# team-charls/charls

Measured on AMD Instinct MI355X. Metric: MPixels/s encode+decode, 4096x4096 8-bit gray, bit-exact vs CharLS, higher is better.
Workload: dtype u8

## Files before the change

charls_amd/csrc/device/pipeline_common.hip:

```cpp
#pragma once
#include <hip/hip_runtime.h>

#include "knobs.h"
#include "scan_model.h"


namespace jls {
namespace pipe {

constexpr int kChains = 367;
constexpr int kRegularChains = 365;
constexpr int kInterruptChain = 365;
constexpr int kZeroContextChain = 366;
constexpr uint32_t kGradientTable = 512;
constexpr uint32_t kNoSlot = 0xFFFFFFFFu;
constexpr uint16_t kNoEvent = 0xFFFF;
constexpr uint32_t kPackBlock = 4096;
constexpr uint32_t kStatusInvalid = 1u;
constexpr uint32_t kChainPad = 16;
constexpr uint32_t kChainSlack = kChains * kChainPad + 64;

struct Work
{
    uint32_t* raw;
    uint64_t raw_words;
    uint64_t* total_bits;
    uint32_t* status;
    uint32_t* stuff_tables;
};

JLS_DEV uint32_t coded_lines(const ScanDesc& d)
{
    return d.interleave_mode == 1 ? d.height * (uint32_t)d.components : d.height;
}
JLS_DEV bool sign_fits_record(const ScanDesc& d)
{
    return d.bits_per_sample <= 15;
}
JLS_DEV uint32_t line_step(const ScanDesc& d)
{
    return d.interleave_mode == 1 ? (uint32_t)d.components : 1u;
}

template <typename S>
JLS_DEV void load_pixel(const ScanDesc& d, uint32_t y, uint32_t x, int mask, int out[4]);

template <typename S, int ILV>
JLS_DEV int load_sample(const ScanDesc& d, uint32_t line, uint32_t x, int mask)
{
    if (ILV == 1)
    {
        int px[4];
        load_pixel<S>(d, line / (uint32_t)d.components, x, mask, px);
        return px[line % (uint32_t)d.components];
    }
    const S* row = reinterpret_cast<const S*>(d.pixels + (size_t)line * d.pixel_stride);
    return (int)row[x] & mask;
}

JLS_DEV uint32_t line_samples(const ScanDesc& d)
{
    return d.interleave_mode == 2 ? d.width * (uint32_t)d.components : d.width;
}

template <typename S>
JLS_DEV void load_pixel(const ScanDesc& d, uint32_t y, uint32_t x, int mask, int out[4])
{
    const S* px = reinterpret_cast<const S*>(d.pixels + (size_t)y * d.pixel_stride) + (size_t)x * d.components;
    for (int c = 0; c < d.components; ++c)
        out[c] = (int)px[c] & mask;
    if (d.color_transformation != 0)
    {
        unsigned t[3];
        hp_forward(d.color_transformation, sizeof(S) == 2, out[0], out[1], out[2], t);
        out[0] = (int)t[0];
        out[1] = (int)t[1];
        out[2] = (int)t[2];
    }
}

typedef uint32_t u32x4 __attribute__((vector_size(16)));

struct CodeWord
{
    uint64_t bits;
    int len;
};

JLS_DEV CodeWord golomb_word(const Traits& t, int k, int m, int limit)
// ... 119 lines not shown
```

charls_amd/csrc/device/scan_model.h:

```cpp
#pragma once
#include <hip/hip_runtime.h>

#include "scan_types.h"

namespace jls {

#define JLS_DEV __device__ __forceinline__

#define JLS_LOCKSTEP() __builtin_amdgcn_wave_barrier()
#ifdef JLS_EMULATED
#define JLS_LOCKSTEP_STORES() __builtin_amdgcn_wave_barrier()
#else
#define JLS_LOCKSTEP_STORES() ((void)0)
#endif

#ifdef JLS_PATH_PROFILE
extern "C" unsigned long long jls_path_counts[32];
#define JLS_PATH(n) do { if (threadIdx.x == 0) ++jls_path_counts[n]; } while (0)
#define JLS_PATH_ADD(n, v) do { if (threadIdx.x == 0) jls_path_counts[n] += (unsigned long long)(v); } while (0)
#else
#define JLS_PATH(n) ((void)0)
#define JLS_PATH_ADD(n, v) ((void)0)
#endif

#ifndef JLS_GLOBAL_AS
#define JLS_GLOBAL_AS __attribute__((address_space(1)))
#endif

#ifndef JLS_DYNAMIC_LDS
#define JLS_DYNAMIC_LDS(name) extern __shared__ __attribute__((aligned(16))) unsigned char name[]
#endif

JLS_DEV uint32_t uniform(uint32_t v)
{
    return (uint32_t)__builtin_amdgcn_readfirstlane((int)v);
}

JLS_DEV uint32_t from_lane(uint32_t v, int l)
{
    return (uint32_t)__builtin_amdgcn_readlane((int)v, l);
}

#ifndef JLS_EMULATED
JLS_DEV int med3(int a, int b, int c)
{
    int r;
    asm("v_med3_i32 %0, %1, %2, %3" : "=v"(r) : "v"(a), "v"(b), "v"(c));
    return r;
}
JLS_DEV int med3s(int a, int b, int c_scalar)
{
    int r;
    asm("v_med3_i32 %0, %1, %2, %3" : "=v"(r) : "v"(a), "v"(b), "s"(c_scalar));
    return r;
}
#else
JLS_DEV int med3(int a, int b, int c)
{
    const int lo = a < b ? a : b, hi = a < b ? b : a;
    return c < lo ? lo : (c > hi ? hi : c);
// ... 112 lines not shown
                 : "s"(busy), "s"(ok)
                 : "scc");
    return ticker;
}
JLS_DEV uint32_t opaque(uint32_t v)
{
    asm volatile("" : "+v"(v));
    return v;
}
JLS_DEV uint32_t float_bits(uint32_t v)
{
    return __float_as_uint((float)v);
}
#define JLS_LDS_AS __attribute__((address_space(3)))
JLS_DEV uint32_t lds_address(const void* p)
{
    return (uint32_t)(uintptr_t)(const JLS_LDS_AS void*)p;
}
template <typename T>
JLS_DEV T lds_load(uint32_t address)
{
    return *(const JLS_LDS_AS T*)(uintptr_t)address;
}
template <typename T>
JLS_DEV void lds_store(uint32_t address, T v)
{
    *(JLS_LDS_AS T*)(uintptr_t)address = v;
}
JLS_DEV uint64_t load_relaxed(const uint64_t* p)
{
    return __hip_atomic_load(p, __ATOMIC_RELAXED, __HIP_MEMORY_SCOPE_AGENT);
}
JLS_DEV void store_relaxed(uint64_t* p, uint64_t v)
{
    __hip_atomic_store(p, v, __ATOMIC_RELAXED, __HIP_MEMORY_SCOPE_AGENT);
}
JLS_DEV uint32_t funnel_shift(uint32_t hi, uint32_t lo, uint32_t shift)
{
    return __builtin_amdgcn_alignbit(hi, lo, shift);
}
#else
JLS_DEV LaneMask lanes_where(bool p)
{
    return __ballot(p);
}
JLS_DEV bool lane_of(LaneMask m)
{
    return ((m >> emu::lane_id()) & 1ull) != 0;
}
JLS_DEV uint32_t value_of_lowest_lane(LaneMask m, uint32_t v)
{
    return (uint32_t)__builtin_amdgcn_readlane((int)v, __builtin_ctzll(m));
}
JLS_DEV int mad24(int a, int b, int c)
{
    return a * b + c;
}
JLS_DEV uint32_t pack_bytes(uint32_t s0, uint32_t s1)
{
    return (s1 & 0xFFu) | ((s0 & 0xFFu) << 8);
}
JLS_DEV uint32_t bit_field(uint32_t v, uint32_t offset, uint32_t width)
{
    return (v >> offset) & ((1u << width) - 1u);
}
JLS_DEV int sign_extend(int v, int bits)
// ... 324 lines not shown
```

charls_amd/csrc/device/tile_pipeline.hip:

```cpp
#pragma once
#include <hip/hip_runtime.h>

#include <algorithm>
#include <cstdlib>

#include "pipeline_common.hip"

namespace jls {
namespace tile {

using pipe::kChains;
using pipe::kInterruptChain;
using pipe::kNoEvent;
using pipe::kStatusInvalid;
using pipe::kZeroContextChain;


constexpr uint32_t kMaxTileSamples = 8192;
constexpr uint32_t kTileLines = 16;
constexpr uint32_t kSegments = 16;
constexpr uint32_t kThreads = 512;
constexpr uint32_t kWaves = kThreads / 64;
constexpr uint32_t kPackThreads = 512;
constexpr uint16_t kNoLocalSlot = 0xFFFF;
// ... 229 lines not shown
            all_a += na;
            all_b += nb;
        }
        a[half] = before_a + incl_a - a[half];
        b[half] = before_b + incl_b - b[half];
        carry_a += all_a;
        carry_b += all_b;
    }
}

template <typename S, int ILV>
struct Samples
{
    const ScanDesc& d;
    const S* rows;
    uint32_t first_line;
    int mask;
    JLS_DEV int operator()(uint32_t line, uint32_t x) const
    {
        static_assert(ILV == 0, "planar scans only");
        return (int)rows[(size_t)(line + 1 - first_line) * d.width + x] & mask;
    }
};

template <typename S, int ILV>
JLS_DEV void stage_lines(const ScanDesc& d, const TileGeometry& g, S* rows)
{
    const uint32_t width = g.width;
    const uint32_t bytes = width * (uint32_t)sizeof(S);
    const uint32_t first = g.first_line == 0 ? 1u : 0u;
    if (first)
        for (uint32_t x = threadIdx.x; x < width; x += blockDim.x)
            rows[x] = 0;
    const uint8_t* from = d.pixels + (size_t)(g.first_line + first - 1) * d.pixel_stride;
    uint8_t* to = reinterpret_cast<uint8_t*>(rows) + (size_t)first * bytes;
    const uint32_t lines = g.tile_lines + 1 - first;
    if (((reinterpret_cast<uintptr_t>(from) | d.pixel_stride | bytes) & 3u) == 0 && (reinterpret_cast<uintptr_t>(to) & 3u) == 0)
    {
        const uint32_t words_per_line = bytes / 4, total = lines * words_per_line;
        constexpr int kMost = (kMaxTileSamples * 2 / 4 + kThreads - 1) / kThreads;
        const uint32_t step_lines = kThreads / words_per_line, step_words = kThreads % words_per_line;
        uint32_t line = threadIdx.x / words_per_line, word = threadIdx.x % words_per_line;
        uint32_t held[kMost];
#pragma unroll
        for (int j = 0; j < kMost; ++j)
        {
            held[j] = line < lines ? reinterpret_cast<const uint32_t*>(from + (size_t)line * d.pixel_stride)[word] : 0u;
            line += step_lines;
            word += step_words;
            if (word >= words_per_line)
            {
                word -= words_per_line;
                ++line;
            }
        }
#pragma unroll
        for (int j = 0; j < kMost; ++j)
        {
            const uint32_t i = threadIdx.x + (uint32_t)j * kThreads;
            if (i < total)
                reinterpret_cast<uint32_t*>(to)[i] = held[j];
        }
        for (uint32_t i = threadIdx.x + kMost * kThreads; i < total; i += kThreads)
        {
            const uint32_t l2 = i / words_per_line, w2 = i - l2 * words_per_line;
            reinterpret_cast<uint32_t*>(to)[i] = reinterpret_cast<const uint32_t*>(from + (size_t)l2 * d.pixel_stride)[w2];
        }
    }
    else
        for (uint32_t r = 0; r < lines; ++r)
        {
            const S* from1 = reinterpret_cast<const S*>(from + (size_t)r * d.pixel_stride);
            S* to1 = reinterpret_cast<S*>(to + (size_t)r * bytes);
            for (uint32_t x = threadIdx.x; x < width; x += blockDim.x)
                to1[x] = from1[x];
        }
}

JLS_HOST_DEV_EARLY uint32_t sort_segments(uint32_t lines_per_tile)
{
    return lines_per_tile >= kWaves ? lines_per_tile : lines_per_tile * (kWaves / lines_per_tile);
}

struct TileLds
{
    uint32_t rows, keys, masks, table, end;
};
template <typename S, int ILV>
JLS_DEV TileLds tile_lds(uint32_t width, uint32_t lines_per_tile, bool with_keys)
{
    auto up = [](uint32_t v) { return (v + 15u) & ~15u; };
    TileLds l;
    const uint32_t chunks = (width + 63) / 64;
    l.rows = 0;
    l.keys = up((lines_per_tile + 1) * width * (uint32_t)sizeof(S));
    l.masks = l.keys + (with_keys ? up(lines_per_tile * width * 2u) : 0u);
    l.table = l.masks + up(lines_per_tile * chunks * 16u);
    l.end = l.table;
    return l;
}

template <typename S, int ILV>
__global__ void __launch_bounds__(kThreads) analyze_tiles(const ScanDesc* __restrict__ descs, const Work* __restrict__ works)
{
    JLS_DYNAMIC_LDS(smem);
// ... 45 lines not shown
                if (y >= step)
                {
                    rb = sample(y - step, x);
                    rc = x > 0 ? sample(y - step, x - 1) : edge_c;
                    rd = sample(y - step, x + 1 < width ? x + 1 : width - 1);
                }
                else
                    rc = x > 0 ? 0 : edge_c;
                const int qs = sizeof(S) == 1
                                   ? ((int)s_grad[rd - rb + 255] * 9 + (int)s_grad[rb - rc + 255]) * 9 + (int)s_grad[rc - ra + 255] - 364
                                   : context_id(t, ra, rb, rc, rd);
                const int sg = qs >> 31;
                const int ctx = (qs ^ sg) - sg;
                s_key[r * width + x] = (uint16_t)(ctx | ((sg & 1) << 9));
                eq = v == ra;
                q0 = qs == 0;
            }
            const unsigned long long m_eq = __ballot(eq);
            const unsigned long long m_q0 = __ballot(q0);
            if (lane == 0)
            {
                s_eq[r * chunks + k] = m_eq;
                s_q0[r * chunks + k] = m_q0;
            }
        }
    }
    __syncthreads();
    for (uint32_t sgm = wave; sgm < g.segments; sgm += kWaves)
    {
        const uint32_t r = sgm / g.pieces, piece = sgm % g.pieces;
        const uint32_t y = g.first_line + r;
        const uint32_t k0 = piece * g.chunks_per_piece;
        const uint32_t k1 = k0 + g.chunks_per_piece < chunks ? k0 + g.chunks_per_piece : chunks;
        uint16_t* key_row = w.keyinv + (size_t)y * width;
        unsigned long long carry = 0;
        for (uint32_t k = 0; k < k1; ++k)
        {
            const unsigned long long a = s_eq[r * chunks + k];
            const unsigned long long b = a & s_q0[r * chunks + k];
            const unsigned long long sum = a + b + carry;
            const unsigned long long st = sum ^ a ^ b;
            carry = (((a & b) | ((a | b) & st)) >> 63) & 1ull;
            const uint32_t x = k * 64 + lane;
            if (k >= k0 && x < width)
            {
                const bool s = (st >> lane) & 1ull;
                const bool q0 = (s_q0[r * chunks + k] >> lane) & 1ull;
                const bool eq = (a >> lane) & 1ull;
                uint16_t key = s_key[r * width + x];
                if (!(s || q0))
                    atomicAdd(&s_hist[key & 0x1FF], 1u);
                else if (s && eq)
                    key = kNoEvent;
                else if (s)
                {
                    key = (uint16_t)kInterruptChain;
                    atomicAdd(&s_hist[kInterruptChain], 1u);
                }
                else
                {
                    key = 0;
                    atomicAdd(&s_hist[0], 1u);
                }
                key_row[x] = key;
            }
        }
    }
    __syncthreads();
    for (uint32_t c = threadIdx.x; c < (uint32_t)kChains; c += kThreads)
        w.seg[(size_t)tile * kChains + c] = s_hist[c];
}

constexpr uint32_t kPlanThreads = 384;
JLS_DEV void plan_group(const ScanDesc& d, const Work& w, uint32_t g, uint32_t& t0, uint32_t& t1)
{
    const uint32_t tiles = scan_tiles(d, w);
    const uint32_t per_group = (tiles + kPlanGroups - 1) / kPlanGroups;
    t0 = g * per_group < tiles ? g * per_group : tiles;
    t1 = t0 + per_group < tiles ? t0 + per_group : tiles;
}
__global__ void __launch_bounds__(kPlanThreads) sum_chains(const ScanDesc* __restrict__ descs, const Work* __restrict__ works)
{
    const ScanDesc d = descs[blockIdx.y];
    const Work w = works[blockIdx.y];
    const uint32_t g = blockIdx.x, c = threadIdx.x;
    if (c >= (uint32_t)kChains)
        return;
    uint32_t t0, t1;
    plan_group(d, w, g, t0, t1);
    uint32_t sum = 0;
    for (uint32_t t = t0; t < t1; ++t)
        sum += w.seg[(size_t)t * kChains + c];
    w.plan_part[g * kChains + c] = sum * (c == 0 ? w.run_slots : 1u);
}
__global__ void __launch_bounds__(kPlanThreads) plan_chains(const ScanDesc* __restrict__ descs, const Work* __restrict__ works)
{
    __shared__ uint32_t s_base[kChains + 1];
    const Work w = works[blockIdx.x];
    uint32_t total = 0;
    if (threadIdx.x < (uint32_t)kChains)
    {
        const uint32_t c = threadIdx.x;
        for (uint32_t g = 0; g < kPlanGroups; ++g)
// ... 96 lines not shown
    static JLS_DEV int which(uint32_t v) { return (int)((v >> (kRunBits + kErrBits)) & 1u); }
    static JLS_DEV uint32_t component(uint32_t v) { return (v >> (is_end_of_line(v) ? 15u : kRunBits + kErrBits + 1)) & 3u; }
};

template <typename S, int ILV>
__global__ void __launch_bounds__(kThreads) sort_tiles(const ScanDesc* __restrict__ descs, const Work* __restrict__ works)
{
    JLS_DYNAMIC_LDS(smem);
    const ScanDesc d = descs[blockIdx.y];
    const Work w = works[blockIdx.y];
    const Traits t = make_traits(d);
    const uint32_t tile = tile_of_block(blockIdx.x, scan_tiles(d, w));
    if (tile >= scan_tiles(d, w))
        return;
    const TileGeometry g = tile_geometry(d, w, tile);
    constexpr uint32_t step = 1;
    const int lane = threadIdx.x & 63, wave = threadIdx.x >> 6;
    const uint32_t width = g.width, chunks = g.chunks;
    const TileLds lds = tile_lds<S, ILV>(width, w.lines_per_tile, false);
    S* s_rows = reinterpret_cast<S*>(smem + lds.rows);
    uint64_t* s_noev = reinterpret_cast<uint64_t*>(smem + lds.masks);
    uint32_t* s_lead = reinterpret_cast<uint32_t*>(s_noev + (size_t)w.lines_per_tile * chunks);
    uint32_t* s_segoff = reinterpret_cast<uint32_t*>(smem + lds.table);
    uint32_t* s_tileoff = s_segoff + sort_segments(w.lines_per_tile) * kChains;
    uint32_t* s_count = s_tileoff + kChains + 1;
    uint32_t* s_global = s_count + kChains + 1;
    uint32_t* s_tmp = s_global + kChains + 1;
    uint32_t* s_same = s_tmp + 16;
    uint32_t* s_rowbase = s_same + kWaves * (kChains + 1);
    uint16_t* s_rowchain = reinterpret_cast<uint16_t*>(s_rowbase + kChains + 1);
    Slot<S>* s_stage = reinterpret_cast<Slot<S>*>(s_rowbase + kChains + 1 + kRowChainWords);
    const int mask = (1 << d.bits_per_sample) - 1;
    const Samples<S, ILV> sample{d, s_rows, g.first_line, mask};
    const uint16_t* key_tile = w.keyinv + (size_t)g.first_line * width;

    JLS_PHASE_BEGIN();
    stage_lines<S, ILV>(d, g, s_rows);
    JLS_PHASE(0);
    for (uint32_t i = threadIdx.x; i < g.segments * (uint32_t)kChains; i += kThreads)
        s_segoff[i] = 0;
    for (uint32_t i = threadIdx.x; i < kWaves * ((uint32_t)kChains + 1); i += kThreads)
        s_same[i] = 0;
    __syncthreads();
    JLS_PHASE(1);
    for (uint32_t sgm = wave; sgm < g.segments; sgm += kWaves)
    {
        const uint32_t r = sgm / g.pieces, piece = sgm % g.pieces;
        const uint32_t k0 = piece * g.chunks_per_piece;
        const uint32_t k1 = k0 + g.chunks_per_piece < chunks ? k0 + g.chunks_per_piece : chunks;
        for (uint32_t kb = k0; kb < k1; kb += 16)
        {
            uint16_t held[16];
#pragma unroll
            for (int j = 0; j < 16; ++j)
            {
                const uint32_t x = (kb + j) * 64 + lane;
                held[j] = kb + j < k1 && x < width ? key_tile[(size_t)r * width + x] : kNoEvent;
            }
#pragma unroll
            for (int j = 0; j < 16; ++j)
            {
                const uint32_t k = kb + j;
                if (k < k1)
                {
                    const uint32_t x = k * 64 + lane;
                    const uint16_t key = held[j];
                    if (x < width && key != kNoEvent)
                        atomicAdd(&s_segoff[sgm * kChains + (key & 0x1FF)], (key & 0x1FF) == 0 ? run_slots_of<S>() : 1u);
                    const unsigned long long m = __ballot(x < width && key == kNoEvent);
                    if (lane == 0)
                        s_noev[r * chunks + k] = m;
                }
            }
        }
    }
    JLS_PHASE(2);
    __syncthreads();
    JLS_PHASE(3);
    for (uint32_t r = (uint32_t)wave; r < g.tile_lines; r += kWaves)
    {
        uint32_t behind = 0;
        for (uint32_t k0 = (chunks - 1) / 64 * 64;; k0 -= 64)
        {
            const uint32_t k = k0 + (uint32_t)lane;
            const unsigned long long m = k < chunks ? s_noev[r * chunks + k] : 0ull;
            const bool full = m == ~0ull;
            const uint32_t own = full ? 64u : (uint32_t)__ffsll(~m) - 1;
            const unsigned long long rest = __ballot(full) >> lane;
            const uint32_t ones = rest == ~0ull ? 64u : (uint32_t)__ffsll(~rest) - 1;
            const uint32_t next = __shfl(own, (int)((lane + ones) & 63u));
            const uint32_t lead = 64u * ones + ((uint32_t)lane + ones < 64u ? next : behind);
            if (k < chunks)
                s_lead[r * (chunks + 1) + k] = lead;
            behind = __shfl(lead, 0);
            if (k0 == 0)
                break;
        }
        if (lane == 0)
            s_lead[r * (chunks + 1) + chunks] = 0;
    }
    {
        static_assert(kChains <= kThreads, "a chain per thread");
        const uint32_t c = threadIdx.x;
        const bool chain = c < (uint32_t)kChains;
        uint32_t n = 0;
        if (chain)
            for (uint32_t sgm = 0; sgm < g.segments; ++sgm)
                n += s_segoff[sgm * kChains + c];
        const uint32_t rows = chain && c != (uint32_t)kInterruptChain ? (n + 63) / 64 : 0u;
        uint32_t off[2] = {n, 0}, row_base[2] = {rows, 0};
        block_exclusive_scan_pair(off, row_base, kChains, s_tmp);
        if (chain)
        {
            s_tileoff[c] = off[0];
            s_count[c] = n;
            s_global[c] = w.seg[(size_t)tile * kChains + c];
            uint32_t running = off[0];
            for (uint32_t sgm = 0; sgm < g.segments; ++sgm)
            {
                const uint32_t m = s_segoff[sgm * kChains + c];
                s_segoff[sgm * kChains + c] = running;
                running += m;
            }
            s_rowbase[c] = row_base[0];
            for (uint32_t j = 0; j < rows; ++j)
                s_rowchain[row_base[0] + j] = (uint16_t)c;
            if (c == (uint32_t)kChains - 1)
                s_rowbase[kChains] = row_base[0] + rows;
        }
    }
    JLS_PHASE(4);
    __syncthreads();
    JLS_PHASE(5);
    for (uint32_t sgm = wave; sgm < g.segments; sgm += kWaves)
    {
        const uint32_t r = sgm / g.pieces, piece = sgm % g.pieces;
        const uint32_t y = g.first_line + r;
        const uint32_t k0 = piece * g.chunks_per_piece;
        const uint32_t k1 = k0 + g.chunks_per_piece < chunks ? k0 + g.chunks_per_piece : chunks;
        uint32_t* segoff = s_segoff + sgm * kChains;
        uint32_t* same_of = s_same + (uint32_t)wave * (kChains + 1);
        uint16_t* inv_row = w.keyinv + (size_t)y * width;
        auto key_at = [&](uint32_t k) -> uint16_t {
            const uint32_t x = k * 64 + lane;
            return k < k1 && x < width ? inv_row[x] : kNoEvent;
        };
        uint16_t key_1 = key_at(k0), key_2 = key_at(k0 + 1);
        const S* cur = s_rows + (r + 1) * width;
        const int edge_a = y >= step ? sample(y - step, 0) : 0;
        const int edge_c = y >= 2 * step ? (r >= 1 ? sample(y - 2 * step, 0) : pipe::load_sample<S, 0>(d, y - 2, 0, mask)) : 0;
        const uint32_t lane_bit = 1u << (lane & 31), below = lane_bit - 1u;
        const bool upper = lane >= 32;
        for (uint32_t k = k0; k < k1; ++k)
        {
            const uint32_t x = k * 64 + lane;
            const bool inside = x < width;
            const uint16_t key = key_1;
            key_1 = key_2;
            key_2 = key_at(k + 2);
            const bool has = key != kNoEvent;
            const uint32_t chain = key & 0x1FFu;
            if (has && !upper)
                atomicOr(&same_of[chain], lane_bit);
            JLS_LOCKSTEP();
            const uint32_t lo = has ? same_of[chain] : 0u;
            JLS_LOCKSTEP();
            if (has && !upper)
                same_of[chain] = 0;
            JLS_LOCKSTEP();
            if (has && upper)
                atomicOr(&same_of[chain], lane_bit);
            JLS_LOCKSTEP();
            const uint32_t hi = has ? same_of[chain] : 0u;
            const uint32_t base = has ? segoff[chain] : 0u;
            JLS_LOCKSTEP();
            if (has && upper)
                same_of[chain] = 0;
            const uint32_t rank = upper ? (uint32_t)__popc(lo) + (uint32_t)__popc(hi & below) : (uint32_t)__popc(lo & below);
            const uint32_t per_event = chain == 0 ? run_slots_of<S>() : 1u;
            if (has && rank == 0)
                segoff[chain] = base + ((uint32_t)__popc(lo) + (uint32_t)__popc(hi)) * per_event;
            JLS_LOCKSTEP();
            const uint32_t slot = base + rank * per_event;
            uint32_t record = 0;
            if (inside)
            {
                const int v = (int)cur[x] & mask;
                const int ra = x > 0 ? (int)cur[x - 1] & mask : edge_a;
                const int rb = (int)(cur - width)[x] & mask;
                const int rc = x > 0 ? (int)(cur - width)[x - 1] & mask : edge_c;
                record = make_record<S>(v, med3(ra + rb - rc, ra, rb), (key >> 9) & 1, t.maxval);
            }
            if (__any(has && chain == 0))
            {
                if (has && chain == 0)
                {
                    const int v = sample(y, x);
                    const int ra = x > 0 ? sample(y, x - 1) : edge_a;
                    uint32_t run = 0;
                    if (v == ra)
                    {
                        const unsigned long long after = lane == 63 ? 0ull : s_noev[r * chunks + k] >> (lane + 1);
                        const uint32_t rest = 63u - (uint32_t)lane;
                        uint32_t n = (uint32_t)__ffsll(~after) - 1;
                        if (n >= rest)
                            n = rest + s_lead[r * (chunks + 1) + k + 1];
                        run = 1 + n;
                    }
                    const uint32_t xi = x + run;
                    if (xi >= width)
                        record = RunRecord<S>::end_of_line(run, 0u);
                    else
                    {
                        const int xv = sample(y, xi);
                        const int ia = xi > 0 ? sample(y, xi - 1) : edge_a;
                        const int ib = y >= step ? sample(y - step, xi) : 0;
                        const int which = ia == ib ? 1 : 0;
                        const int err = which ? error_value(t, xv - ia) : error_value(t, (xv - ib) * ((ib - ia) < 0 ? -1 : 1));
                        record = RunRecord<S>::interrupted(run, err, which, 0u);
                    }
                }
            }
            if (has)
            {
                if (run_slots_of<S>() == 2 && chain == 0)
                {
                    s_stage[slot] = (Slot<S>)(record & 0xFFFFu);
                    s_stage[slot + 1] = (Slot<S>)(record >> 16);
                }
                else
                    s_stage[slot] = (Slot<S>)record;
            }
            if (inside)
                inv_row[x] = has ? (uint16_t)slot : kNoLocalSlot;
        }
    }
    JLS_PHASE(6);
    __syncthreads();
    JLS_PHASE(7);
    const uint32_t total_rows = s_rowbase[kChains];
    constexpr int kRows = 4;
    for (uint32_t q0 = (uint32_t)wave * kRows; q0 < total_rows; q0 += kWaves * kRows)
    {
        uint32_t to[kRows];
        Slot<S> held[kRows];
        bool live[kRows];
#pragma unroll
        for (int j = 0; j < kRows; ++j)
        {
            const uint32_t q = q0 + (uint32_t)j;
            const uint32_t c = q < total_rows ? s_rowchain[q] : 0u;
            const uint32_t i = (q - s_rowbase[c]) * 64 + (uint32_t)lane;
            live[j] = q < total_rows && i < s_count[c];
            to[j] = s_global[c] + i;
            held[j] = live[j] ? s_stage[s_tileoff[c] + i] : (Slot<S>)0;
        }
#pragma unroll
        for (int j = 0; j < kRows; ++j)
            if (live[j])
                rec_slots<S>(w)[to[j]] = held[j];
    }
    JLS_PHASE(8);
}

}
}
#include "tile_pixel_mode.hip"
namespace jls {
namespace tile {

struct Chain
{
    int a, b, c, n;
    uint32_t bad;
};

JLS_DEV int chain_n_before(uint32_t i, uint32_t reset)
{
    if (reset == 0 || i < reset)
        return (int)(i + 1);
    const uint32_t half = reset >> 1, period = reset - half;
    return (int)(half + 1 + (i - reset) % period);
}

template <typename S>
JLS_DEV Slot<S> code_event(Chain& s, uint32_t rec, const Traits& t)
{
    int err;
    if (sizeof(S) == 1)
    {
        const int px = med3(s.c + (int)(rec >> 8), 0, t.maxval);
        err = sign_extend((int)(rec & 0xFFu) - px, t.bpp);
    }
// ... 792 lines not shown
    const uint32_t codes = (uint32_t)stage_bytes(tile_capacity, sample_bytes);
    const uint32_t head = ((codes + 3u) & ~3u) + 4 * ((uint32_t)kChains + 1) * 4 + kPackThreads * 4 + 16 * 4 + kRowChainWords * 4;
    return (head + 15u) & ~15u;
}

JLS_HOST_DEV uint32_t pack_bits_words(uint32_t tile_capacity, int32_t bits_per_sample)
{
    const uint32_t limit = 2u * (uint32_t)(bits_per_sample + (bits_per_sample > 8 ? bits_per_sample : 8));
    return tile_capacity * limit / 32 + 2;
}

JLS_DEV void expand_code(uint32_t word, uint64_t& bits, int& len)
{
    if (word & kRunTag)
    {
        const int ones = (int)((word >> 25) & 63u), tail_len = (int)((word >> 20) & 31u);
        bits = ((((uint64_t)1 << ones) - 1ull) << tail_len) | (uint64_t)(word & 0xFFFFFu);
        len = ones + tail_len;
    }
    else
    {
        bits = word & 0xFFFFFFu;
        len = (int)(word >> 24);
    }
}

JLS_DEV uint32_t shifted_word(const uint32_t* bits, uint32_t i, uint32_t head, uint32_t carry)
{
    if (head == 0)
        return bits[i];
    return (i == 0 ? carry : bits[i - 1] << (32u - head)) | (bits[i] >> head);
}

struct __attribute__((packed)) UnalignedQuadPair
{
    uint64_t lo, hi;
};
template <typename S>
__global__ void __launch_bounds__(kPackThreads) pack_tiles(const ScanDesc* __restrict__ descs, const Work* __restrict__ works)
{
    JLS_DYNAMIC_LDS(smem);
    constexpr bool kNarrow = sizeof(Slot<S>) == 2;
    const ScanDesc d = descs[blockIdx.y];
    const Work w = works[blockIdx.y];
    const uint32_t tile = blockIdx.x;
    const uint32_t tiles = scan_tiles(d, w);
    if (tile >= tiles)
        return;
    const uint32_t tile_capacity = w.tile_capacity;
    const uint32_t threads = blockDim.x;
    const uint32_t per_thread = ((tile_capacity + threads - 1) / threads + 7u) & ~7u;
    const int lane = threadIdx.x & 63, wave = threadIdx.x >> 6;
    const uint32_t kPackWaves = threads / 64;
    Slot<S>* s_code = reinterpret_cast<Slot<S>*>(smem);
    const uint32_t code_bytes = (uint32_t)stage_bytes(tile_capacity, (uint32_t)sizeof(S));
    uint32_t* s_tileoff = reinterpret_cast<uint32_t*>(smem + ((code_bytes + 3u) & ~3u));
    uint32_t* s_count = s_tileoff + kChains + 1;
    uint32_t* s_global = s_count + kChains + 1;
    uint32_t* s_scan = s_global + kChains + 1;
    uint32_t* s_tmp = s_scan + kPackThreads;
    uint32_t* s_rowbase = s_tmp + 16;
    uint16_t* s_rowchain = reinterpret_cast<uint16_t*>(s_rowbase + kChains + 1);
    uint32_t* s_bits = reinterpret_cast<uint32_t*>(smem + pack_bits_offset(tile_capacity, (uint32_t)sizeof(S)));
    const TileSpan span = tile_span(d, w, tile);
    const uint32_t tile_samples = span.count;
    const uint16_t* inv = w.keyinv + span.first;

    constexpr int kGroups = (int)(kMaxTileSamples / kPackThreads / 8);
    uint4 mine[kGroups];
    JLS_PHASE_BEGIN();
#pragma unroll
    for (int q = 0; q < kGroups; ++q)
    {
        const uint32_t at = threadIdx.x * per_thread + (uint32_t)q * 8;
        mine[q] = make_uint4(~0u, ~0u, ~0u, ~0u);
        if ((uint32_t)q * 8 < per_thread && at + 8 <= tile_samples)
        {
            const UnalignedQuadPair v = *reinterpret_cast<const UnalignedQuadPair*>(inv + at);
            mine[q] = make_uint4((uint32_t)v.lo, (uint32_t)(v.lo >> 32), (uint32_t)v.hi, (uint32_t)(v.hi >> 32));
        }
        else if ((uint32_t)q * 8 < per_thread && at < tile_samples)
        {
            uint32_t e[8];
#pragma unroll
            for (int j = 0; j < 8; ++j)
                e[j] = at + (uint32_t)j < tile_samples ? inv[at + j] : kNoLocalSlot;
            mine[q] = make_uint4(e[0] | (e[1] << 16), e[2] | (e[3] << 16), e[4] | (e[5] << 16), e[6] | (e[7] << 16));
        }
    }
    {
        uint32_t n[2] = {0, 0}, g[2] = {0, 0}, rows[2] = {0, 0};
        for (int half = 0; half < 2; ++half)
        {
            const uint32_t c = threadIdx.x + (uint32_t)half * threads;
            if (c < (uint32_t)kChains)
            {
                g[half] = w.seg[(size_t)tile * kChains + c];
                n[half] = w.seg[(size_t)(tile + 1) * kChains + c] - g[half];
                rows[half] = (n[half] + 63) / 64;
            }
        }
        uint32_t off[2] = {n[0], n[1]}, row_base[2] = {rows[0], rows[1]};
        block_exclusive_scan_pair(off, row_base, kChains, s_tmp);
        for (int half = 0; half < 2; ++half)
        {
            const uint32_t c = threadIdx.x + (uint32_t)half * threads;
            if (c < (uint32_t)kChains)
            {
                s_tileoff[c] = off[half];
                s_count[c] = n[half];
                s_global[c] = g[half];
                s_rowbase[c] = row_base[half];
                for (uint32_t j = 0; j < rows[half]; ++j)
                    s_rowchain[row_base[half] + j] = (uint16_t)c;
                if (c == (uint32_t)kChains - 1)
                    s_rowbase[kChains] = row_base[half] + rows[half];
            }
        }
    }
    JLS_PHASE(9);
    __syncthreads();
    JLS_PHASE(11);
    {
        const uint32_t total_rows = s_rowbase[kChains];
        constexpr int kRows = 16;
        for (uint32_t q0 = (uint32_t)wave * kRows; q0 < total_rows; q0 += kPackWaves * kRows)
        {
            uint32_t to[kRows];
            Slot<S> held[kRows];
            bool live[kRows];
#pragma unroll
            for (int j = 0; j < kRows; ++j)
            {
                const uint32_t q = q0 + (uint32_t)j;
                const uint32_t c = q < total_rows ? s_rowchain[q] : 0u;
                const uint32_t i = (q - s_rowbase[c]) * 64 + (uint32_t)lane;
                live[j] = q < total_rows && i < s_count[c];
                to[j] = s_tileoff[c] + i;
                held[j] = live[j] ? code_slots<S>(w)[s_global[c] + i] : (Slot<S>)0;
            }
#pragma unroll
            for (int j = 0; j < kRows; ++j)
                if (live[j])
                    s_code[to[j]] = held[j];
        }
    }
    JLS_PHASE(12);
    __syncthreads();
    JLS_PHASE(13);

    auto slot_of = [&](int q, int j) -> uint32_t {
        const uint32_t word = (j >> 1) == 0 ? mine[q].x : (j >> 1) == 1 ? mine[q].y : (j >> 1) == 2 ? mine[q].z : mine[q].w;
        return (j & 1) ? word >> 16 : word & 0xFFFFu;
    };
    const uint32_t run_slots_end = kNarrow ? s_count[0] : 0u;
    auto word_of = [&](uint32_t slot) -> uint32_t {
        if (slot == kNoLocalSlot)
            return 0u;
        if (!kNarrow)
            return (uint32_t)s_code[slot];
        if (slot < run_slots_end)
            return (uint32_t)s_code[slot] | ((uint32_t)s_code[slot + 1] << 16);
        const uint32_t c = (uint32_t)s_code[slot];
        return ((c >> 10) << 24) | (c & 0x3FFu);
    };
    uint32_t words[kGroups * 8];
    uint32_t sum = 0;
#pragma unroll
    for (int q = 0; q < kGroups; ++q)
#pragma unroll
        for (int j = 0; j < 8; ++j)
        {
            const uint32_t word = word_of(slot_of(q, j));
            words[q * 8 + j] = word;
            sum += word & kRunTag ? ((word >> 25) & 63u) + ((word >> 20) & 31u) : word >> 24;
        }
    JLS_PHASE(14);
    {
        uint32_t incl = sum;
        for (int delta = 1; delta < 64; delta <<= 1)
        {
            const uint32_t up = __shfl_up(incl, delta);
            if (lane >= delta)
                incl += up;
        }
        if (lane == 63)
            s_tmp[wave] = incl;
        __syncthreads();
        uint32_t before = 0;
        for (uint32_t w2 = 0; w2 < kPackWaves; ++w2)
            before += (int)w2 < wave ? s_tmp[w2] : 0u;
        s_scan[threadIdx.x] = before + incl;
        __syncthreads();
    }
    JLS_PHASE(15);
    const uint32_t tile_bits = s_scan[threads - 1];
    if (threadIdx.x == 0)
        store_relaxed(&w.blockbase[tile], (tile == 0 ? pipe::kBlockUpTo : pipe::kBlockOwn) | (uint64_t)tile_bits);
    const uint32_t local_words = (tile_bits + 31) / 32;
    for (uint32_t i = threadIdx.x; i < local_words + 1; i += threads)
        s_bits[i] = 0;
    __syncthreads();
    if (sum != 0)
    {
        const uint32_t bitpos = s_scan[threadIdx.x] - sum;
        uint32_t word_at = bitpos >> 5;
        const uint32_t first_word = word_at;
        uint32_t pending = bitpos & 31;
        uint64_t acc = 0;
        auto put = [&](uint32_t part, uint32_t n) {
            acc |= (uint64_t)part << ((64u - pending - n) & 63u);
            pending += n;
            if (pending >= 32)
            {
                const uint32_t o = (uint32_t)(acc >> 32);
                if (word_at == first_word)
                    atomicOr(&s_bits[word_at], o);
                else
                    s_bits[word_at] = o;
                acc <<= 32;
                pending -= 32;
                ++word_at;
            }
        };
#pragma unroll
        for (int q = 0; q < kGroups; ++q)
#pragma unroll
            for (int j = 0; j < 8; ++j)
            {
                const uint32_t word = words[q * 8 + j];
                if (word == 0)
                    continue;
                uint64_t v;
                int len;
                expand_code(word, v, len);
                if (len > 32)
                {
                    put((uint32_t)(v >> 32), (uint32_t)len - 32u);
                    len = 32;
                }
                put((uint32_t)v, (uint32_t)len);
            }
        if (pending > 0)
            atomicOr(&s_bits[word_at], (uint32_t)(acc >> 32));
    }
    JLS_PHASE(18);
    __syncthreads();
    JLS_PHASE(19);
    const bool last_tile = tile + 1 == tiles;
    constexpr uint64_t kTailValid = 1ull << 63;
    if (threadIdx.x < 64)
    {
        const uint64_t own = tile_bits;
        const uint32_t b = tile;
        uint64_t start = 0;
        uint32_t reach = b;
        while (reach > 0)
        {
            const bool in_window = (uint32_t)lane < reach;
            const uint32_t j = in_window ? reach - 1 - (uint32_t)lane : 0;
            uint64_t state = 0;
            do
            {
                state = in_window ? load_relaxed(&w.blockbase[j]) : pipe::kBlockOwn;
            } while (__any((state >> 62) == 0));
            const unsigned long long knows = __ballot(in_window && (state >> 62) == 2);
            const int last = knows ? (int)__ffsll(knows) - 1 : 63;
            uint64_t part = in_window && lane <= last ? state & pipe::kBlockValue : 0;
            for (int delta = 32; delta > 0; delta >>= 1)
                part += __shfl_xor(part, delta);
            start += part;
            if (knows)
                break;
            reach = reach > 64 ? reach - 64 : 0;
        }
        if (lane == 0)
        {
            if (b != 0)
                store_relaxed(&w.blockbase[b], pipe::kBlockUpTo | (start + own));
            if (b + 1 == tiles)
                *w.total_bits = start + own;
            const uint32_t head = (uint32_t)(start & 31);
            const uint32_t tile_words = (head + tile_bits + 31) / 32;
            const bool shared_first = head != 0;
            const bool partial_last = ((head + tile_bits) & 31u) != 0 && !last_tile;
            const bool own_tail = tile_words >= 2 || !shared_first;
            if (own_tail)
                store_relaxed(&w.tile_tail[tile], kTailValid | (partial_last ? shifted_word(s_bits, tile_words - 1, head, 0u) : 0u));
            uint32_t carry = 0;
            if (shared_first)
            {
                uint64_t before;
                do
                    before = load_relaxed(&w.tile_tail[tile - 1]);
                while ((before & kTailValid) == 0);
                carry = (uint32_t)before;
            }
            if (!own_tail)
                store_relaxed(&w.tile_tail[tile], kTailValid | (partial_last ? shifted_word(s_bits, 0, head, carry) : 0u));
            s_tmp[12] = (uint32_t)start;
            s_tmp[13] = (uint32_t)(start >> 32);
            s_tmp[14] = carry;
        }
    }
    JLS_PHASE(16);
    __syncthreads();
    JLS_PHASE(20);
    const uint64_t tile_start = (uint64_t)s_tmp[12] | ((uint64_t)s_tmp[13] << 32);
    const uint32_t head = (uint32_t)(tile_start & 31), carry = s_tmp[14];
    const uint32_t tile_words = (head + tile_bits + 31) / 32;
    const bool partial_last = ((head + tile_bits) & 31u) != 0 && !last_tile;
    const uint64_t first_global = tile_start >> 5;
    const uint32_t stored_words = partial_last ? tile_words - 1 : tile_words;
    for (uint32_t i = threadIdx.x; i < stored_words; i += threads)
    {
        const uint64_t at = first_global + i;
        if (at < w.raw_words)
            w.raw[at] = __builtin_bswap32(shifted_word(s_bits, i, head, carry));
    }
    if (last_tile && threadIdx.x < 4)
    {
        const uint64_t at = first_global + tile_words + threadIdx.x;
        if (at < w.raw_words)
            w.raw[at] = 0;
    }
    JLS_PHASE(21);
}

__global__ void __launch_bounds__(256) clear_pack_state(const Work* __restrict__ works, uint32_t bytes_per_scan)
{
    uint4* at = reinterpret_cast<uint4*>(works[blockIdx.y].blockbase);
    const uint32_t groups = bytes_per_scan / 16;
    for (uint32_t g = blockIdx.x * 256u + threadIdx.x; g < groups; g += gridDim.x * 256u)
        at[g] = make_uint4(0, 0, 0, 0);
}

inline size_t tile_common_lds_bytes(uint32_t width, uint32_t lines_per_tile, uint32_t sample_bytes, int interleave_mode, bool with_keys)
{
    auto up = [](size_t v) { return (v + 15) & ~size_t{15}; };
    const size_t chunks = (width + 63) / 64;
    return up(interleave_mode == 1 ? 0 : (size_t)(lines_per_tile + 1) * width * sample_bytes) +
           (with_keys ? up((size_t)lines_per_tile * width * 2) : 0) + up((size_t)lines_per_tile * chunks * 16);
}
inline size_t analyze_lds_bytes(uint32_t width, uint32_t lines_per_tile, uint32_t sample_bytes, int interleave_mode)
{
    return tile_common_lds_bytes(width, lines_per_tile, sample_bytes, interleave_mode, true) + ((size_t)kChains + 1) * 4 + pipe::kGradientTable;
}
inline size_t sort_lds_bytes(uint32_t width, uint32_t lines_per_tile, uint32_t sample_bytes, int interleave_mode)
{
    return tile_common_lds_bytes(width, lines_per_tile, sample_bytes, interleave_mode, false) + (size_t)sort_segments(lines_per_tile) * kChains * 4 +
           4 * ((size_t)kChains + 1) * 4 + 16 * 4 + (size_t)kWaves * (kChains + 1) * 4 + kRowChainWords * 4 +
           stage_bytes((uint32_t)lines_per_tile * width, sample_bytes);
}
inline uint32_t pack_threads_for(uint32_t tile_capacity)
{
    const uint32_t per_thread = ((tile_capacity + kPackThreads - 1) / kPackThreads + 7u) & ~7u;
    if ((uint64_t)per_thread * kPackThreads * 4 <= (uint64_t)tile_capacity * 5)
// ... 52 lines not shown
```

Baseline: 16670.

## Use global address space pointers and split run-record computation from key staging

Casts device pointers to the global address space so the compiler can emit global rather than flat loads and stores. In the tile planning kernel, key rows are fetched once into packed registers and reused across both passes when segments fit, and inverse-slot writes are batched per 16 chunks. Run-interruption records are now computed in a separate lane-parallel pass over the run slots instead of inside the per-chunk loop. This adds register pressure and a second pass, in exchange for fewer divergent branches and less repeated key traffic.

```diff
diff --git a/charls_amd/csrc/device/pipeline_common.hip b/charls_amd/csrc/device/pipeline_common.hip
--- a/charls_amd/csrc/device/pipeline_common.hip
+++ b/charls_amd/csrc/device/pipeline_common.hip
@@ -54,7 +54,7 @@
         load_pixel<S>(d, line / (uint32_t)d.components, x, mask, px);
         return px[line % (uint32_t)d.components];
     }
-    const S* row = reinterpret_cast<const S*>(d.pixels + (size_t)line * d.pixel_stride);
+    const auto row = reinterpret_cast<const JLS_GLOBAL_AS S*>(global_ptr(d.pixels) + (size_t)line * d.pixel_stride);
     return (int)row[x] & mask;
 }
 
diff --git a/charls_amd/csrc/device/scan_model.h b/charls_amd/csrc/device/scan_model.h
--- a/charls_amd/csrc/device/scan_model.h
+++ b/charls_amd/csrc/device/scan_model.h
@@ -26,6 +26,11 @@
 #ifndef JLS_GLOBAL_AS
 #define JLS_GLOBAL_AS __attribute__((address_space(1)))
 #endif
+template <typename T>
+JLS_DEV JLS_GLOBAL_AS T* global_ptr(T* p)
+{
+    return (JLS_GLOBAL_AS T*)p;
+}
 
 #ifndef JLS_DYNAMIC_LDS
 #define JLS_DYNAMIC_LDS(name) extern __shared__ __attribute__((aligned(16))) unsigned char name[]
@@ -204,6 +209,14 @@
     return __hip_atomic_load(p, __ATOMIC_RELAXED, __HIP_MEMORY_SCOPE_AGENT);
 }
 JLS_DEV void store_relaxed(uint64_t* p, uint64_t v)
+{
+    __hip_atomic_store(p, v, __ATOMIC_RELAXED, __HIP_MEMORY_SCOPE_AGENT);
+}
+JLS_DEV uint64_t load_relaxed(const JLS_GLOBAL_AS uint64_t* p)
+{
+    return __hip_atomic_load(p, __ATOMIC_RELAXED, __HIP_MEMORY_SCOPE_AGENT);
+}
+JLS_DEV void store_relaxed(JLS_GLOBAL_AS uint64_t* p, uint64_t v)
 {
     __hip_atomic_store(p, v, __ATOMIC_RELAXED, __HIP_MEMORY_SCOPE_AGENT);
 }
diff --git a/charls_amd/csrc/device/tile_pipeline.hip b/charls_amd/csrc/device/tile_pipeline.hip
--- a/charls_amd/csrc/device/tile_pipeline.hip
+++ b/charls_amd/csrc/device/tile_pipeline.hip
@@ -285,7 +285,7 @@
     if (first)
         for (uint32_t x = threadIdx.x; x < width; x += blockDim.x)
             rows[x] = 0;
-    const uint8_t* from = d.pixels + (size_t)(g.first_line + first - 1) * d.pixel_stride;
+    const auto from = global_ptr(d.pixels) + (size_t)(g.first_line + first - 1) * d.pixel_stride;
     uint8_t* to = reinterpret_cast<uint8_t*>(rows) + (size_t)first * bytes;
     const uint32_t lines = g.tile_lines + 1 - first;
     if (((reinterpret_cast<uintptr_t>(from) | d.pixel_stride | bytes) & 3u) == 0 && (reinterpret_cast<uintptr_t>(to) & 3u) == 0)
@@ -298,7 +298,7 @@
 #pragma unroll
         for (int j = 0; j < kMost; ++j)
         {
-            held[j] = line < lines ? reinterpret_cast<const uint32_t*>(from + (size_t)line * d.pixel_stride)[word] : 0u;
+            held[j] = line < lines ? reinterpret_cast<const JLS_GLOBAL_AS uint32_t*>(from + (size_t)line * d.pixel_stride)[word] : 0u;
             line += step_lines;
             word += step_words;
             if (word >= words_per_line)
@@ -317,13 +317,13 @@
         for (uint32_t i = threadIdx.x + kMost * kThreads; i < total; i += kThreads)
         {
             const uint32_t l2 = i / words_per_line, w2 = i - l2 * words_per_line;
-            reinterpret_cast<uint32_t*>(to)[i] = reinterpret_cast<const uint32_t*>(from + (size_t)l2 * d.pixel_stride)[w2];
+            reinterpret_cast<uint32_t*>(to)[i] = reinterpret_cast<const JLS_GLOBAL_AS uint32_t*>(from + (size_t)l2 * d.pixel_stride)[w2];
         }
     }
     else
         for (uint32_t r = 0; r < lines; ++r)
         {
-            const S* from1 = reinterpret_cast<const S*>(from + (size_t)r * d.pixel_stride);
+            const auto from1 = reinterpret_cast<const JLS_GLOBAL_AS S*>(from + (size_t)r * d.pixel_stride);
             S* to1 = reinterpret_cast<S*>(to + (size_t)r * bytes);
             for (uint32_t x = threadIdx.x; x < width; x += blockDim.x)
                 to1[x] = from1[x];
@@ -435,7 +435,7 @@
         const uint32_t y = g.first_line + r;
         const uint32_t k0 = piece * g.chunks_per_piece;
         const uint32_t k1 = k0 + g.chunks_per_piece < chunks ? k0 + g.chunks_per_piece : chunks;
-        uint16_t* key_row = w.keyinv + (size_t)y * width;
+        const auto key_row = global_ptr(w.keyinv) + (size_t)y * width;
         unsigned long long carry = 0;
         for (uint32_t k = 0; k < k1; ++k)
         {
@@ -471,7 +471,7 @@
     }
     __syncthreads();
     for (uint32_t c = threadIdx.x; c < (uint32_t)kChains; c += kThreads)
-        w.seg[(size_t)tile * kChains + c] = s_hist[c];
+        global_ptr(w.seg)[(size_t)tile * kChains + c] = s_hist[c];
 }
 
 constexpr uint32_t kPlanThreads = 384;
@@ -634,7 +634,7 @@
     Slot<S>* s_stage = reinterpret_cast<Slot<S>*>(s_rowbase + kChains + 1 + kRowChainWords);
     const int mask = (1 << d.bits_per_sample) - 1;
     const Samples<S, ILV> sample{d, s_rows, g.first_line, mask};
-    const uint16_t* key_tile = w.keyinv + (size_t)g.first_line * width;
+    const auto key_tile = global_ptr(w.keyinv) + (size_t)g.first_line * width;
 
     JLS_PHASE_BEGIN();
     stage_lines<S, ILV>(d, g, s_rows);
@@ -645,6 +645,27 @@
         s_same[i] = 0;
     __syncthreads();
     JLS_PHASE(1);
+    const bool keys_kept = g.segments <= kWaves && g.chunks_per_piece <= 16;
+    uint32_t keys2[8];
+#pragma unroll
+    for (int i = 0; i < 8; ++i)
+        keys2[i] = 0xFFFFFFFFu;
+    auto fetch_keys = [&](uint32_t r, uint32_t kb, uint32_t k1) {
+        uint32_t held[16];
+#pragma unroll
+        for (int j = 0; j < 16; ++j)
+        {
+            const uint32_t x = (kb + j) * 64 + lane;
+            held[j] = key_tile[(size_t)r * width + (x < width ? x : width - 1)];
+        }
+#pragma unroll
+        for (int j = 0; j < 16; ++j)
+            if (!(kb + j < k1 && (kb + j) * 64 + lane < width))
+                held[j] = kNoEvent;
+#pragma unroll
+        for (int i = 0; i < 8; ++i)
+            keys2[i] = held[2 * i] | (held[2 * i + 1] << 16);
+    };
     for (uint32_t sgm = wave; sgm < g.segments; sgm += kWaves)
     {
         const uint32_t r = sgm / g.pieces, piece = sgm % g.pieces;
@@ -652,24 +673,17 @@
         const uint32_t k1 = k0 + g.chunks_per_piece < chunks ? k0 + g.chunks_per_piece : chunks;
         for (uint32_t kb = k0; kb < k1; kb += 16)
         {
-            uint16_t held[16];
-#pragma unroll
-            for (int j = 0; j < 16; ++j)
-            {
-                const uint32_t x = (kb + j) * 64 + lane;
-                held[j] = kb + j < k1 && x < width ? key_tile[(size_t)r * width + x] : kNoEvent;
-            }
+            fetch_keys(r, kb, k1);
 #pragma unroll
             for (int j = 0; j < 16; ++j)
             {
                 const uint32_t k = kb + j;
                 if (k < k1)
                 {
-                    const uint32_t x = k * 64 + lane;
-                    const uint16_t key = held[j];
-                    if (x < width && key != kNoEvent)
+                    const uint16_t key = (uint16_t)(keys2[j >> 1] >> ((j & 1) * 16));
+                    if (key != kNoEvent)
                         atomicAdd(&s_segoff[sgm * kChains + (key & 0x1FF)], (key & 0x1FF) == 0 ? run_slots_of<S>() : 1u);
-                    const unsigned long long m = __ballot(x < width && key == kNoEvent);
+                    const unsigned long long m = __ballot(k * 64 + lane < width && key == kNoEvent);
                     if (lane == 0)
                         s_noev[r * chunks + k] = m;
                 }
@@ -716,7 +730,7 @@
         {
             s_tileoff[c] = off[0];
             s_count[c] = n;
-            s_global[c] = w.seg[(size_t)tile * kChains + c];
+            s_global[c] = global_ptr(w.seg)[(size_t)tile * kChains + c];
             uint32_t running = off[0];
             for (uint32_t sgm = 0; sgm < g.segments; ++sgm)
             {
@@ -742,90 +756,111 @@
         const uint32_t k1 = k0 + g.chunks_per_piece < chunks ? k0 + g.chunks_per_piece : chunks;
         uint32_t* segoff = s_segoff + sgm * kChains;
         uint32_t* same_of = s_same + (uint32_t)wave * (kChains + 1);
-        uint16_t* inv_row = w.keyinv + (size_t)y * width;
-        auto key_at = [&](uint32_t k) -> uint16_t {
-            const uint32_t x = k * 64 + lane;
-            return k < k1 && x < width ? inv_row[x] : kNoEvent;
-        };
-        uint16_t key_1 = key_at(k0), key_2 = key_at(k0 + 1);
+        const auto inv_row = key_tile + (size_t)r * width;
         const S* cur = s_rows + (r + 1) * width;
         const int edge_a = y >= step ? sample(y - step, 0) : 0;
         const int edge_c = y >= 2 * step ? (r >= 1 ? sample(y - 2 * step, 0) : pipe::load_sample<S, 0>(d, y - 2, 0, mask)) : 0;
         const uint32_t lane_bit = 1u << (lane & 31), below = lane_bit - 1u;
         const bool upper = lane >= 32;
-        for (uint32_t k = k0; k < k1; ++k)
-        {
-            const uint32_t x = k * 64 + lane;
-            const bool inside = x < width;
-            const uint16_t key = key_1;
-            key_1 = key_2;
-            key_2 = key_at(k + 2);
-            const bool has = key != kNoEvent;
-            const uint32_t chain = key & 0x1FFu;
-            if (has && !upper)
-                atomicOr(&same_of[chain], lane_bit);
-            JLS_LOCKSTEP();
-            const uint32_t lo = has ? same_of[chain] : 0u;
-            JLS_LOCKSTEP();
-            if (has && !upper)
-                same_of[chain] = 0;
-            JLS_LOCKSTEP();
-            if (has && upper)
-                atomicOr(&same_of[chain], lane_bit);
-            JLS_LOCKSTEP();
-            const uint32_t hi = has ? same_of[chain] : 0u;
-            const uint32_t base = has ? segoff[chain] : 0u;
-            JLS_LOCKSTEP();
-            if (has && upper)
-                same_of[chain] = 0;
-            const uint32_t rank = upper ? (uint32_t)__popc(lo) + (uint32_t)__popc(hi & below) : (uint32_t)__popc(lo & below);
-            const uint32_t per_event = chain == 0 ? run_slots_of<S>() : 1u;
-            if (has && rank == 0)
-                segoff[chain] = base + ((uint32_t)__popc(lo) + (uint32_t)__popc(hi)) * per_event;
-            JLS_LOCKSTEP();
-            const uint32_t slot = base + rank * per_event;
-            uint32_t record = 0;
-            if (inside)
-            {
-                const int v = (int)cur[x] & mask;
-                const int ra = x > 0 ? (int)cur[x - 1] & mask : edge_a;
-                const int rb = (int)(cur - width)[x] & mask;
-                const int rc = x > 0 ? (int)(cur - width)[x - 1] & mask : edge_c;
-                record = make_record<S>(v, med3(ra + rb - rc, ra, rb), (key >> 9) & 1, t.maxval);
-            }
-            if (__any(has && chain == 0))
-            {
-                if (has && chain == 0)
+        const uint32_t run_first = segoff[0];
+        for (uint32_t kb = k0; kb < k1; kb += 16)
+        {
+            if (!keys_kept)
+                fetch_keys(r, kb, k1);
+            const uint32_t batch = k1 - kb < 16u ? k1 - kb : 16u;
+            for (uint32_t j = 0; j < 16; ++j)
+            {
+                uint32_t out = kNoLocalSlot;
+                if (j < batch)
                 {
-                    const int v = sample(y, x);
-                    const int ra = x > 0 ? sample(y, x - 1) : edge_a;
-                    uint32_t run = 0;
-                    if (v == ra)
+                    const uint32_t x = (kb + j) * 64 + lane;
+                    const bool inside = x < width;
+                    const uint32_t key = keys2[0] & 0xFFFFu;
+                    const bool has = key != kNoEvent;
+                    const uint32_t chain = key & 0x1FFu;
+                    if (has && !upper)
+                        atomicOr(&same_of[chain], lane_bit);
+                    JLS_LOCKSTEP();
+                    const uint32_t lo = has ? same_of[chain] : 0u;
+                    JLS_LOCKSTEP();
+                    if (has && !upper)
+                        same_of[chain] = 0;
+                    JLS_LOCKSTEP();
+                    if (has && upper)
+                        atomicOr(&same_of[chain], lane_bit);
+                    JLS_LOCKSTEP();
+                    const uint32_t hi = has ? same_of[chain] : 0u;
+                    const uint32_t base = has ? segoff[chain] : 0u;
+                    JLS_LOCKSTEP();
+                    if (has && upper)
+                        same_of[chain] = 0;
+                    const uint32_t rank = upper ? (uint32_t)__popc(lo) + (uint32_t)__popc(hi & below) : (uint32_t)__popc(lo & below);
+                    const uint32_t per_event = chain == 0 ? run_slots_of<S>() : 1u;
+                    if (has && rank == 0)
+                        segoff[chain] = base + ((uint32_t)__popc(lo) + (uint32_t)__popc(hi)) * per_event;
+                    JLS_LOCKSTEP();
+                    const uint32_t slot = base + rank * per_event;
+                    uint32_t record = 0;
+                    if (inside)
                     {
-                        const unsigned long long after = lane == 63 ? 0ull : s_noev[r * chunks + k] >> (lane + 1);
-                        const uint32_t rest = 63u - (uint32_t)lane;
-                        uint32_t n = (uint32_t)__ffsll(~after) - 1;
-                        if (n >= rest)
-                            n = rest + s_lead[r * (chunks + 1) + k + 1];
-                        run = 1 + n;
+                        const int v = (int)cur[x] & mask;
+                        const int ra = x > 0 ? (int)cur[x - 1] & mask : edge_a;
+                        const int rb = (int)(cur - width)[x] & mask;
+                        const int rc = x > 0 ? (int)(cur - width)[x - 1] & mask : edge_c;
+                        record = make_record<S>(v, med3(ra + rb - rc, ra, rb), (key >> 9) & 1, t.maxval);
                     }
-                    const uint32_t xi = x + run;
-                    if (xi >= width)
-                        record = RunRecord<S>::end_of_line(run, 0u);
-                    else
-                    {
-                        const int xv = sample(y, xi);
-                        const int ia = xi > 0 ? sample(y, xi - 1) : edge_a;
-                        const int ib = y >= step ? sample(y - step, xi) : 0;
-                        const int which = ia == ib ? 1 : 0;
-                        const int err = which ? error_value(t, xv - ia) : error_value(t, (xv - ib) * ((ib - ia) < 0 ? -1 : 1));
-                        record = RunRecord<S>::interrupted(run, err, which, 0u);
-                    }
+                    if (has)
+                        s_stage[slot] = (Slot<S>)(chain == 0 ? x : record);
+                    out = has ? slot : (uint32_t)kNoLocalSlot;
                 }
-            }
-            if (has)
-            {
-                if (run_slots_of<S>() == 2 && chain == 0)
+#pragma unroll
+                for (int i = 0; i < 7; ++i)
+                    keys2[i] = (keys2[i] >> 16) | (keys2[i + 1] << 16);
+                keys2[7] = (keys2[7] >> 16) | (out << 16);
+            }
+#pragma unroll
+            for (int j = 0; j < 16; ++j)
+            {
+                const uint32_t x = (kb + j) * 64 + lane;
+                if (kb + j < k1 && x < width)
+                    inv_row[x] = (uint16_t)(keys2[j >> 1] >> ((j & 1) * 16));
+            }
+        }
+        JLS_LOCKSTEP();
+        const uint32_t run_end = segoff[0];
+        for (uint32_t first = run_first; first < run_end; first += 64 * run_slots_of<S>())
+        {
+            const uint32_t slot = first + (uint32_t)lane * run_slots_of<S>();
+            if (slot < run_end)
+            {
+                const uint32_t x = (uint32_t)s_stage[slot];
+                const uint32_t k = x >> 6, bit = x & 63u;
+                const int v = sample(y, x);
+                const int ra = x > 0 ? sample(y, x - 1) : edge_a;
+                uint32_t run = 0;
+                if (v == ra)
+                {
+                    const unsigned long long after = bit == 63 ? 0ull : s_noev[r * chunks + k] >> (bit + 1);
+                    const uint32_t rest = 63u - bit;
+                    uint32_t n = (uint32_t)__ffsll(~after) - 1;
+                    if (n >= rest)
+                        n = rest + s_lead[r * (chunks + 1) + k + 1];
+                    run = 1 + n;
+                }
+                const uint32_t xi = x + run;
+                uint32_t record;
+                if (xi >= width)
+                    record = RunRecord<S>::end_of_line(run, 0u);
+                else
+                {
+                    const int xv = sample(y, xi);
+                    const int ia = xi > 0 ? sample(y, xi - 1) : edge_a;
+                    const int ib = y >= step ? sample(y - step, xi) : 0;
+                    const int which = ia == ib ? 1 : 0;
+                    const int err = which ? error_value(t, xv - ia) : error_value(t, (xv - ib) * ((ib - ia) < 0 ? -1 : 1));
+                    record = RunRecord<S>::interrupted(run, err, which, 0u);
+                }
+                if (run_slots_of<S>() == 2)
                 {
                     s_stage[slot] = (Slot<S>)(record & 0xFFFFu);
                     s_stage[slot + 1] = (Slot<S>)(record >> 16);
@@ -833,8 +868,6 @@
                 else
                     s_stage[slot] = (Slot<S>)record;
             }
-            if (inside)
-                inv_row[x] = has ? (uint16_t)slot : kNoLocalSlot;
         }
     }
     JLS_PHASE(6);
@@ -860,7 +893,7 @@
 #pragma unroll
         for (int j = 0; j < kRows; ++j)
             if (live[j])
-                rec_slots<S>(w)[to[j]] = held[j];
+                global_ptr(rec_slots<S>(w))[to[j]] = held[j];
     }
     JLS_PHASE(8);
 }
@@ -1719,10 +1752,7 @@
     return (i == 0 ? carry : bits[i - 1] << (32u - head)) | (bits[i] >> head);
 }
 
-struct __attribute__((packed)) UnalignedQuadPair
-{
-    uint64_t lo, hi;
-};
+typedef uint32_t UnalignedWords4 __attribute__((vector_size(16), aligned(2)));
 template <typename S>
 __global__ void __launch_bounds__(kPackThreads) pack_tiles(const ScanDesc* __restrict__ descs, const Work* __restrict__ works)
 {
@@ -1751,7 +1781,7 @@
     uint32_t* s_bits = reinterpret_cast<uint32_t*>(smem + pack_bits_offset(tile_capacity, (uint32_t)sizeof(S)));
     const TileSpan span = tile_span(d, w, tile);
     const uint32_t tile_samples = span.count;
-    const uint16_t* inv = w.keyinv + span.first;
+    const auto inv = global_ptr(w.keyinv) + span.first;
 
     constexpr int kGroups = (int)(kMaxTileSamples / kPackThreads / 8);
     uint4 mine[kGroups];
@@ -1763,8 +1793,8 @@
         mine[q] = make_uint4(~0u, ~0u, ~0u, ~0u);
         if ((uint32_t)q * 8 < per_thread && at + 8 <= tile_samples)
         {
-            const UnalignedQuadPair v = *reinterpret_cast<const UnalignedQuadPair*>(inv + at);
-            mine[q] = make_uint4((uint32_t)v.lo, (uint32_t)(v.lo >> 32), (uint32_t)v.hi, (uint32_t)(v.hi >> 32));
+            const UnalignedWords4 v = *reinterpret_cast<const JLS_GLOBAL_AS UnalignedWords4*>(inv + at);
+            mine[q] = make_uint4(v[0], v[1], v[2], v[3]);
         }
         else if ((uint32_t)q * 8 < per_thread && at < tile_samples)
         {
@@ -1782,8 +1812,8 @@
             const uint32_t c = threadIdx.x + (uint32_t)half * threads;
             if (c < (uint32_t)kChains)
             {
-                g[half] = w.seg[(size_t)tile * kChains + c];
-                n[half] = w.seg[(size_t)(tile + 1) * kChains + c] - g[half];
+                g[half] = global_ptr(w.seg)[(size_t)tile * kChains + c];
+                n[half] = global_ptr(w.seg)[(size_t)(tile + 1) * kChains + c] - g[half];
                 rows[half] = (n[half] + 63) / 64;
             }
         }
@@ -1824,7 +1854,7 @@
                 const uint32_t i = (q - s_rowbase[c]) * 64 + (uint32_t)lane;
                 live[j] = q < total_rows && i < s_count[c];
                 to[j] = s_tileoff[c] + i;
-                held[j] = live[j] ? code_slots<S>(w)[s_global[c] + i] : (Slot<S>)0;
+                held[j] = live[j] ? global_ptr(code_slots<S>(w))[s_global[c] + i] : (Slot<S>)0;
             }
 #pragma unroll
             for (int j = 0; j < kRows; ++j)
@@ -1883,7 +1913,7 @@
     JLS_PHASE(15);
     const uint32_t tile_bits = s_scan[threads - 1];
     if (threadIdx.x == 0)
-        store_relaxed(&w.blockbase[tile], (tile == 0 ? pipe::kBlockUpTo : pipe::kBlockOwn) | (uint64_t)tile_bits);
+        store_relaxed(&global_ptr(w.blockbase)[tile], (tile == 0 ? pipe::kBlockUpTo : pipe::kBlockOwn) | (uint64_t)tile_bits);
     const uint32_t local_words = (tile_bits + 31) / 32;
     for (uint32_t i = threadIdx.x; i < local_words + 1; i += threads)
         s_bits[i] = 0;
@@ -1949,7 +1979,7 @@
             uint64_t state = 0;
             do
             {
-                state = in_window ? load_relaxed(&w.blockbase[j]) : pipe::kBlockOwn;
+                state = in_window ? load_relaxed(&global_ptr(w.blockbase)[j]) : pipe::kBlockOwn;
             } while (__any((state >> 62) == 0));
             const unsigned long long knows = __ballot(in_window && (state >> 62) == 2);
             const int last = knows ? (int)__ffsll(knows) - 1 : 63;
@@ -1964,27 +1994,27 @@
         if (lane == 0)
         {
             if (b != 0)
-                store_relaxed(&w.blockbase[b], pipe::kBlockUpTo | (start + own));
+                store_relaxed(&global_ptr(w.blockbase)[b], pipe::kBlockUpTo | (start + own));
             if (b + 1 == tiles)
-                *w.total_bits = start + own;
+                *global_ptr(w.total_bits) = start + own;
             const uint32_t head = (uint32_t)(start & 31);
             const uint32_t tile_words = (head + tile_bits + 31) / 32;
             const bool shared_first = head != 0;
             const bool partial_last = ((head + tile_bits) & 31u) != 0 && !last_tile;
             const bool own_tail = tile_words >= 2 || !shared_first;
             if (own_tail)
-                store_relaxed(&w.tile_tail[tile], kTailValid | (partial_last ? shifted_word(s_bits, tile_words - 1, head, 0u) : 0u));
+                store_relaxed(&global_ptr(w.tile_tail)[tile], kTailValid | (partial_last ? shifted_word(s_bits, tile_words - 1, head, 0u) : 0u));
             uint32_t carry = 0;
             if (shared_first)
             {
                 uint64_t before;
                 do
-                    before = load_relaxed(&w.tile_tail[tile - 1]);
+                    before = load_relaxed(&global_ptr(w.tile_tail)[tile - 1]);
                 while ((before & kTailValid) == 0);
                 carry = (uint32_t)before;
             }
             if (!own_tail)
-                store_relaxed(&w.tile_tail[tile], kTailValid | (partial_last ? shifted_word(s_bits, 0, head, carry) : 0u));
+                store_relaxed(&global_ptr(w.tile_tail)[tile], kTailValid | (partial_last ? shifted_word(s_bits, 0, head, carry) : 0u));
             s_tmp[12] = (uint32_t)start;
             s_tmp[13] = (uint32_t)(start >> 32);
             s_tmp[14] = carry;
@@ -2003,13 +2033,13 @@
     {
         const uint64_t at = first_global + i;
         if (at < w.raw_words)
-            w.raw[at] = __builtin_bswap32(shifted_word(s_bits, i, head, carry));
+            global_ptr(w.raw)[at] = __builtin_bswap32(shifted_word(s_bits, i, head, carry));
     }
     if (last_tile && threadIdx.x < 4)
     {
         const uint64_t at = first_global + tile_words + threadIdx.x;
         if (at < w.raw_words)
-            w.raw[at] = 0;
+            global_ptr(w.raw)[at] = 0;
     }
     JLS_PHASE(21);
 }
```

New measurement: 16950 (median of 6 runs). 1.02x the previous value.
